# mjmj531/isaacgym

Measured on AMD Instinct MI355X. Metric: env-steps/sec at N_envs=16384 (1/2/4/8 GPUs) + achieved HBM GB/s vs roofline, higher is better.
Workload: dtype f32; 1 GPU; humanoid_pingpong 3-actor tilt (HumanoidPingpongTiltG1), num_envs=16384 per GPU, random U(-1,1) actions, 2 physics substeps per step, fused step kernel; variant=TT, kind=step, num_envs_per_gpu=16384, global_envs=16384, horizon_stats_every=32, prewarm_launches=512, full=False, launch=HIP graph of 32 steps, replayed, parallelism=env-shard x1, no data-path collective

## Files before the change

__graft_entry__.py:

```python
import os
import sys

ROOT = os.path.dirname(os.path.abspath(__file__))
if ROOT not in sys.path:
    sys.path.insert(0, ROOT)


def build():
    from isaacgym_amd import _lib
    _lib.build(force=False)
    from oracle import binding as oracle_binding
    oracle_binding.build()
    sys.path.insert(0, os.path.join(ROOT, "tests"))
    import shim_binding
    shim_binding.lib()
    import dr_shim_binding
    dr_shim_binding.lib()
    import play_shim_binding
    play_shim_binding.lib()
    import ppo_meter_shim_binding
    ppo_meter_shim_binding.lib()
    import urdf_assets
    urdf_assets.build_second_arm_library()
    urdf_assets.build_second_ta_library()
    import isaacgym_amd
    L = _lib.lib()
    from isaacgym_amd import scene
    assert L.ppenv_abi_version() == scene.ABI_VERSION


def smoke():
    import numpy as np
    import torch
    from isaacgym_amd import _lib, scene
    from isaacgym_amd.env import PPEnv
    from oracle import binding as oracle_binding
    sys.path.insert(0, os.path.join(ROOT, "tests"))
    import helpers

    assert torch.cuda.is_available(), "smoke() needs the GPU box"
    _lib.lib()
    n = 256
    cfg = scene.build_config("TT", num_envs=n, seed=1)
    env = PPEnv(scene.build_config("TT", num_envs=n, seed=1), device="cuda:0")
    ora = oracle_binding.OracleEnv(cfg)
    probe = helpers.SensitivityProbe(oracle_binding, cfg)
    oa, ra = helpers.obs_atol(), helpers.reward_atol(cfg)
    rng = np.random.default_rng(0)
    excluded = 0
    for t in range(8):
        a = rng.uniform(-1, 1, (n, 7)).astype(np.float32)
        st = ora.get_state()
        env.set_state(st)
        ora.step(a)
        env.step(torch.from_numpy(a).cuda())
        torch.cuda.synchronize()
        keep = ~probe.sensitive(st, a, ora)
        excluded += int((~keep).sum())
        assert np.array_equal(env.reset_buf.cpu().numpy()[keep], ora.reset_buf[keep])
        helpers.assert_close(env.obs_buf.cpu().numpy()[keep], ora.obs_buf[keep], f"smoke: obs, step {t}", atol=oa)
        helpers.assert_close(env.rew_buf.cpu().numpy()[keep], ora.rew_buf[keep], f"smoke: rew, step {t}", atol=ra)
    assert excluded <= 4, excluded
    assert env.status == 0
    env.close()
    print(f"smoke ok: fused HIP step matches the CPU oracle on {n} envs x 8 steps (rtol 1e-4, the tests' atol; {excluded} env-steps on a switch set aside)")


if __name__ == "__main__":
    build()
    if len(sys.argv) > 1 and sys.argv[1] == "smoke":
        smoke()
```

isaacgym_amd/csrc/ppenv.hip:

```cpp
#include <hip/hip_runtime.h>

#include <algorithm>
#include <cstdio>
#include <cstdlib>
#include <cstring>
#include <new>

using std::min;
using std::max;

#if defined(PP_STAMP)
__device__ unsigned long long pp_stamp_buf[4096 * 32];
#endif
#include "ppenv_device.h"
#include "ppenv_host.h"

using namespace pp;

namespace {

constexpr int kBlock = 64;
constexpr int kObsStride = PPENV_NUM_OBS + 1;
constexpr int kMaxSplitSubsteps = 4;

struct DevBuffers {
    float* obs;
    float* rew;
    long long* reset;
    long long* progress;
    float* dof_pos;
    float* dof_vel;
    float* dof_force;
    float* ball;
    uint32_t* flags;
    uint32_t* episode;
    float* serve;
};

template <class V>
__device__ __forceinline__ void st_state(V* p, V v) { __builtin_nontemporal_store(v, p); }

template <int A>
__device__ __forceinline__ void load_state(const DevBuffers& b, int n, int i, EnvStateT<A>& st) {
#pragma unroll
    for (int d = 0; d < A * ND; d++) {
        st.q[d] = b.dof_pos[(size_t)d * n + i];
        st.qd[d] = b.dof_vel[(size_t)d * n + i];
    }
    float bl[13];
#pragma unroll
    for (int k = 0; k < 13; k++) bl[k] = b.ball[(size_t)k * n + i];
    st.ball.p = mk(bl[0], bl[1], bl[2]);
#pragma unroll
    for (int k = 0; k < 4; k++) st.ball.quat[k] = bl[3 + k];
    st.ball.v = mk(bl[7], bl[8], bl[9]);
    st.ball.w = mk(bl[10], bl[11], bl[12]);
    st.progress = b.progress[(size_t)i * A];
#pragma unroll
    for (int a = 0; a < A; a++) st.flags[a] = b.flags[(size_t)a * n + i];
    st.episode = b.episode[i];
}
__device__ __forceinline__ void store_ball(const DevBuffers& b, int n, int i, const Ball& ball) {
    const float bl[13] = {ball.p.x, ball.p.y, ball.p.z, ball.quat[0], ball.quat[1], ball.quat[2], ball.quat[3],
                          ball.v.x, ball.v.y, ball.v.z, ball.w.x, ball.w.y, ball.w.z};
#pragma unroll
    for (int k = 0; k < 13; k++) st_state(&b.ball[(size_t)k * n + i], bl[k]);
}
template <int A>
__device__ __forceinline__ void store_task(const DevBuffers& b, int n, int i, const EnvStateT<A>& st, const float* rew, long long reset) {
#pragma unroll
    for (int a = 0; a < A; a++) {
        st_state(&b.progress[(size_t)i * A + a], st.progress);
        st_state(&b.flags[(size_t)a * n + i], st.flags[a]);
        st_state(&b.rew[(size_t)i * A + a], rew[a]);
        st_state(&b.reset[(size_t)i * A + a], reset);
    }
    st_state(&b.episode[i], st.episode);
}
template <int A>
__device__ __forceinline__ void store_state(const DevBuffers& b, int n, int i, const EnvStateT<A>& st, const float* rew, long long reset) {
#pragma unroll
    for (int d = 0; d < A * ND; d++) {
        b.dof_pos[(size_t)d * n + i] = st.q[d];
        b.dof_vel[(size_t)d * n + i] = st.qd[d];
        b.dof_force[(size_t)d * n + i] = st.dof_force[d];
    }
    store_ball(b, n, i, st.ball);
    store_task<A>(b, n, i, st, rew, reset);
}

struct LdsRowStore {
    float* row;
    __device__ __forceinline__ void operator()(int k, float v) { row[k] = v; }
};
struct NoisyRowStore {
    float* row;
    float sigma;
    uint64_t seed;
    uint32_t gid, episode, progress;
    uint32_t base = 16u;
    __device__ __forceinline__ void operator()(int k, float v) { row[k] = v + sigma * dr_gauss(seed, gid, episode, progress, base + (uint32_t)k); }
};
struct DRTables {
    const float* kp; const float* kd; const float* ms; const float* es; const float* fs;
    float act_sigma, obs_sigma;
};

__device__ __forceinline__ void flush_obs(const float* s_obs, float* obs, int base, int nvalid, int lane) {
    const int total = nvalid * PPENV_NUM_OBS;
    float4* dst = reinterpret_cast<float4*>(obs + (size_t)base * PPENV_NUM_OBS);
    for (int k = lane * 4; k < total; k += kBlock * 4) {
        int r = k / PPENV_NUM_OBS, c = k - r * PPENV_NUM_OBS;
        const float* src = &s_obs[r * kObsStride + c];
        typedef float f4v __attribute__((ext_vector_type(4)));
        f4v val = {src[0], src[1], src[2], src[3]};
        __builtin_nontemporal_store(val, reinterpret_cast<f4v*>(&dst[k >> 2]));
    }
}

template <class T, bool DR = false>
__global__ __launch_bounds__(kBlock) void step_kernel(const StepConsts K, DevBuffers b, const float* __restrict__ actions, int serve_on, const DRTables drt = DRTables{}) {
    __shared__ float s_obs[kBlock * kObsStride];
    const int lane = threadIdx.x;
    PP_STAMP_AT(0);
    const int n = K.num_envs;
    const int base = blockIdx.x * kBlock;
    const int i = base + lane;
    const int nvalid = min(kBlock, n - base);

    const bool active = i < n;
    EnvState st;
    float rew = 0.f;
    long long reset = 0;
    if (active) {
        float act[ND];
#pragma unroll
        for (int d = 0; d < ND; d++) act[d] = actions[(size_t)i * ND + d];
        load_state<1>(b, n, i, st);
#if defined(PP_STAMP)
        asm volatile("s_waitcnt vmcnt(0) lgkmcnt(0)" ::: "memory");
#endif
        PP_STAMP_AT(1);
        BodyState bodies[NB];
        float pre_vx;
        EnvDR dr;
        const uint32_t gid = (uint32_t)(K.env_id_offset + i), ep0 = st.episode;
        if (DR) {
#pragma unroll
            for (int d = 0; d < ND; d++) {
                dr.kp[d] = drt.kp ? drt.kp[(size_t)d * n + i] : 1.f;
                dr.kd[d] = drt.kd ? drt.kd[(size_t)d * n + i] : 1.f;
                dr.ms[d] = drt.ms ? drt.ms[(size_t)d * n + i] : 1.f;
            }
            dr.es = drt.es ? drt.es[i] : 1.f;
            dr.fs = drt.fs ? drt.fs[i] : 1.f;
            dr.act_sigma = drt.act_sigma; dr.obs_sigma = drt.obs_sigma;
            dr.key_progress = (uint32_t)st.progress;
        }
        simulate_env<T, 1, DR>(K, act, st, bodies, pre_vx, &dr, gid);
        V3 ov = mk(0, 0, 0);
        if (serve_on) ov = mk(b.serve[i], b.serve[(size_t)n + i], b.serve[2 * (size_t)n + i]);
        LdsRowStore store{&s_obs[lane * kObsStride]};
        NoisyRowStore nstore{&s_obs[lane * kObsStride], dr.obs_sigma, K.seed, gid, ep0, dr.key_progress};
        if (DR && drt.obs_sigma > 0.f) post_physics_env<1>(K, gid, st, bodies, pre_vx, serve_on ? &ov : nullptr, &rew, reset, &nstore);
        else post_physics_env<1>(K, gid, st, bodies, pre_vx, serve_on ? &ov : nullptr, &rew, reset, &store);
// ... 855 lines not shown
        hipLaunchKernelGGL((step_kernel_split<ModelG1, 1, 0>), grid, dim3(2 * kBlock), 0, st, e->K, buf, actions_dev, e->serve_on, e->status.dev, e->dbg_drop_handoff);
        break;
    case SCH_FUSED:
        hipLaunchKernelGGL((step_kernel<ModelG1, false>), grid, dim3(kBlock), 0, st, e->K, buf, actions_dev, e->serve_on, DRTables{});
        break;
    }
    PP_HIP(hipGetLastError());
    return PPENV_OK;
}

const char* ppenv_step_kernel_name(ppenv* e) { return e ? kScheduleNames[schedule_of(e)] : ""; }

int ppenv_step(ppenv* e, const float* actions_dev, void* stream) { return launch_step(e, e ? e->buf : DevBuffers{}, actions_dev, stream); }

int ppenv_step_sequence(ppenv* e, const float* const* actions_dev, int32_t count, void* stream) {
    if (!e || !actions_dev || count < 0) { ppenv_set_error("NULL argument or negative count"); return PPENV_EINVAL; }
    for (int32_t i = 0; i < count; i++)
        if (int rc = launch_step(e, e->buf, actions_dev[i], stream)) return rc;
    return PPENV_OK;
}

int ppenv_step_into(ppenv* e, const float* actions_dev, float* obs_dev, float* rew_dev, int64_t* reset_dev, void* stream) {
    if (!e) { ppenv_set_error("NULL argument"); return PPENV_EINVAL; }
    if (obs_dev && (reinterpret_cast<uintptr_t>(obs_dev) & 15)) { ppenv_set_error("ppenv_step_into: obs must be 16-byte aligned"); return PPENV_EINVAL; }
    DevBuffers b = e->buf;
    if (obs_dev) b.obs = obs_dev;
    if (rew_dev) b.rew = rew_dev;
    if (reset_dev) b.reset = reinterpret_cast<long long*>(reset_dev);
    return launch_step(e, b, actions_dev, stream);
}

int ppenv_reset_all(ppenv* e, void* stream) {
    if (!e) { ppenv_set_error("NULL argument"); return PPENV_EINVAL; }
    if (int rc = check_status(e)) return rc;
    if (int rc = pp_use_device(e->cfg.device_id)) return rc;
    launch_init(e, 1, e->serve_on, (hipStream_t)stream);
    PP_HIP(hipGetLastError());
    return PPENV_OK;
}

uint32_t ppenv_status(ppenv* e) { return e ? e->status.read() : 0u; }

int ppenv_set_randomization(ppenv* e, const ppenv_randomization* dr) {
    if (!e) { ppenv_set_error("NULL argument"); return PPENV_EINVAL; }
    if (!dr) { e->dr_on = 0; e->dr = DRTables{}; return PPENV_OK; }
    if (!(dr->action_noise_sigma >= 0.f) || !(dr->observation_noise_sigma >= 0.f)) { ppenv_set_error("noise amplitudes must be >= 0"); return PPENV_EINVAL; }
    e->dr = DRTables{dr->dof_stiffness_scale, dr->dof_damping_scale, dr->link_mass_scale, dr->restitution_scale, dr->friction_scale,
                     dr->action_noise_sigma, dr->observation_noise_sigma};
    e->dr_on = 1;
    return PPENV_OK;
}

int ppenv_set_gravity(ppenv* e, float gravity_z) {
    if (!e) { ppenv_set_error("NULL argument"); return PPENV_EINVAL; }
    if (!(gravity_z <= 0.f)) { ppenv_set_error("gravity_z must be <= 0 (the world's up axis is z)"); return PPENV_EINVAL; }
    e->cfg.gravity_z = gravity_z;
    e->K = make_step_consts(e->cfg);
    return PPENV_OK;
}

int ppenv_reset_idx(ppenv* e, const int64_t* env_ids_dev, int32_t count, int refresh_obs, void* stream) {
    if (!e || (count > 0 && !env_ids_dev) || count < 0) { ppenv_set_error("ppenv_reset_idx: NULL ids or negative count"); return PPENV_EINVAL; }
    if (count == 0) return PPENV_OK;
    if (int rc = check_status(e)) return rc;
    if (int rc = pp_use_device(e->cfg.device_id)) return rc;
    const dim3 grid((count + kBlock - 1) / kBlock), block(kBlock);
    if (e->agents == 2)
        hipLaunchKernelGGL((reset_idx_kernel<ModelG1, 2>), grid, block, 0, (hipStream_t)stream, e->K, e->buf, (const long long*)env_ids_dev, count, refresh_obs, e->serve_on, e->status.dev);
    else
        hipLaunchKernelGGL((reset_idx_kernel<ModelG1, 1>), grid, block, 0, (hipStream_t)stream, e->K, e->buf, (const long long*)env_ids_dev, count, refresh_obs, e->serve_on, e->status.dev);
    PP_HIP(hipGetLastError());
    return PPENV_OK;
}

int ppenv_pd_targets(ppenv* e, const float* actions_dev, float* pd_tar_dev, void* stream) {
    if (!e || !actions_dev || !pd_tar_dev) { ppenv_set_error("NULL argument"); return PPENV_EINVAL; }
    if (int rc = pp_use_device(e->cfg.device_id)) return rc;
    const int rows = e->cfg.num_envs * e->agents;
    hipLaunchKernelGGL(pd_targets_kernel<ModelG1>, dim3((rows * ND + 255) / 256), dim3(256), 0, (hipStream_t)stream, rows, e->K.clip_actions, actions_dev, pd_tar_dev);
    PP_HIP(hipGetLastError());
    return PPENV_OK;
}

int ppenv_serve_from_draws(ppenv* e, const float* draws_dev, int32_t m, float* vel_dev, void* stream) {
    if (!e || !draws_dev || !vel_dev || m <= 0) { ppenv_set_error("NULL argument or m <= 0"); return PPENV_EINVAL; }
    if (int rc = pp_use_device(e->cfg.device_id)) return rc;
    hipLaunchKernelGGL(serve_from_draws_kernel, dim3((m + 255) / 256), dim3(256), 0, (hipStream_t)stream, e->cfg.variant, m, draws_dev, vel_dev);
    PP_HIP(hipGetLastError());
    return PPENV_OK;
}

int ppenv_reduce_stats(ppenv* e, double* out_dev, void* stream) {
    if (!e || !out_dev) { ppenv_set_error("NULL argument"); return PPENV_EINVAL; }
    if (int rc = check_status(e)) return rc;
    if (int rc = pp_use_device(e->cfg.device_id)) return rc;
    const int rows = e->cfg.num_envs * e->agents;
    if (rows <= 32768) {
        hipLaunchKernelGGL(stats_kernel_single, dim3(1), dim3(1024), 0, (hipStream_t)stream, rows, e->agents, e->buf.rew, e->buf.progress,
                           e->buf.episode, out_dev);
    } else {
        PP_HIP(hipMemsetAsync(out_dev, 0, 4 * sizeof(double), (hipStream_t)stream));
        const int blocks = min(256, (rows + 255) / 256);
        hipLaunchKernelGGL(stats_kernel, dim3(blocks), dim3(256), 0, (hipStream_t)stream, rows, e->agents, e->buf.rew, e->buf.progress,
                           e->buf.episode, out_dev);
    }
    PP_HIP(hipGetLastError());
    return PPENV_OK;
}

int ppenv_post_physics_step(ppenv* e, const float* rigid_body_states_dev, float* root_states_dev, float* dof_states_dev,
                            const float* dof_force_dev, const float* pre_ball_vx_dev, void* stream) {
    if (!e || !rigid_body_states_dev || !root_states_dev || !dof_states_dev || !dof_force_dev || !pre_ball_vx_dev) {
        ppenv_set_error("NULL argument");
        return PPENV_EINVAL;
    }
    if (e->agents != 1) { ppenv_set_error("ppenv_post_physics_step serves the 3-actor variants; the 4-actor entry is ppenv_t4_rewards"); return PPENV_EINVAL; }
    if (int rc = check_status(e)) return rc;
    if (int rc = pp_use_device(e->cfg.device_id)) return rc;
    hipLaunchKernelGGL(post_physics_kernel, dim3(grid_for(e->cfg.num_envs)), dim3(kBlock), 0, (hipStream_t)stream, e->K, e->buf,
                       rigid_body_states_dev, root_states_dev, dof_states_dev, dof_force_dev, pre_ball_vx_dev, e->serve_on);
    PP_HIP(hipGetLastError());
    return PPENV_OK;
}

static int refresh(ppenv* e, float* out, void* stream, void (*kernel)(const StepConsts, DevBuffers, float*), int block) {
    if (!e || !out) { ppenv_set_error("NULL argument"); return PPENV_EINVAL; }
    if (int rc = pp_use_device(e->cfg.device_id)) return rc;
    hipLaunchKernelGGL(kernel, dim3((e->cfg.num_envs + block - 1) / block), dim3(block), 0, (hipStream_t)stream, e->K, e->buf, out);
    PP_HIP(hipGetLastError());
    return PPENV_OK;
}
int ppenv_refresh_root_states(ppenv* e, float* out, void* stream) { return refresh(e, out, stream, refresh_root_kernel, 256); }
int ppenv_refresh_dof_states(ppenv* e, float* out, void* stream) { return refresh(e, out, stream, refresh_dof_kernel, 256); }
int ppenv_refresh_dof_force(ppenv* e, float* out, void* stream) { return refresh(e, out, stream, refresh_dof_force_kernel, 256); }
int ppenv_refresh_rigid_body_states(ppenv* e, float* out, void* stream) { return refresh(e, out, stream, refresh_rb_kernel<ModelG1>, kBlock); }

int ppenv_set_serve_override(ppenv* e, const float* serve_dev, int on, void* stream) {
    if (!e) { ppenv_set_error("NULL argument"); return PPENV_EINVAL; }
    if (int rc = pp_use_device(e->cfg.device_id)) return rc;
    if (on && serve_dev) {
        hipLaunchKernelGGL(serve_transpose_kernel, dim3((e->cfg.num_envs + 255) / 256), dim3(256), 0, (hipStream_t)stream, e->cfg.num_envs,
                           serve_dev, e->buf.serve);
        PP_HIP(hipGetLastError());
    }
    e->serve_on = on ? 1 : 0;
    return PPENV_OK;
}

#if defined(PP_STAMP)
int ppenv_debug_read_stamps(unsigned long long* dst, size_t count) {
    if (hipDeviceSynchronize() != hipSuccess) return PPENV_EHIP;
    return hipMemcpyFromSymbol(dst, HIP_SYMBOL(pp_stamp_buf), count * sizeof(unsigned long long)) == hipSuccess ? 0 : PPENV_EHIP;
}
#endif

size_t ppenv_state_bytes(ppenv* e) {
    if (!e) return 0;
    const size_t A = (size_t)e->agents;
    return (size_t)e->cfg.num_envs * ((A * ND * 3 + 13) * 4 + A * 4 + 4 + A * 8 + A * 8);
}

static int state_io(ppenv* e, char* blob, size_t nbytes, bool to_host) {
    if (!e || !blob) { ppenv_set_error("NULL argument"); return PPENV_EINVAL; }
    if (nbytes != ppenv_state_bytes(e)) { ppenv_set_error("state blob size does not match this handle"); return PPENV_ESTATE; }
    if (int rc = pp_use_device(e->cfg.device_id)) return rc;
    PP_HIP(hipDeviceSynchronize());
    if (int rc = check_status(e)) return rc;
    const size_t n = (size_t)e->cfg.num_envs, A = (size_t)e->agents;
    struct Part { void* dev; size_t bytes; };
    const Part parts[] = {{e->buf.dof_pos, n * A * ND * 4}, {e->buf.dof_vel, n * A * ND * 4}, {e->buf.dof_force, n * A * ND * 4}, {e->buf.ball, n * 13 * 4},
                          {e->buf.flags, n * A * 4}, {e->buf.episode, n * 4}, {e->buf.progress, n * A * 8}, {e->buf.reset, n * A * 8}};
    for (const Part& p : parts) {
        if (to_host) PP_HIP(hipMemcpy(blob, p.dev, p.bytes, hipMemcpyDeviceToHost));
        else PP_HIP(hipMemcpy(p.dev, blob, p.bytes, hipMemcpyHostToDevice));
        blob += p.bytes;
    }
    return PPENV_OK;
}
int ppenv_get_state(ppenv* e, void* dst_host, size_t n) { return state_io(e, (char*)dst_host, n, true); }
int ppenv_set_state(ppenv* e, const void* src_host, size_t n) { return state_io(e, (char*)src_host, n, false); }

}
```

isaacgym_amd/csrc/ppenv_device.h:

```cpp
#pragma once

#include <math.h>
#include <stddef.h>
#include <stdint.h>
#include <string.h>

#include "../../include/ppenv.h"

#if defined(__HIPCC__)
#define PP_HD __host__ __device__ __forceinline__
#else
#define PP_HD inline __attribute__((always_inline))
#endif

#if defined(PP_STAMP) && defined(__HIP_DEVICE_COMPILE__)
#define PP_STAMP_AT(k)                                                                      \
    do {                                                                                    \
        __builtin_amdgcn_sched_barrier(0);                                                  \
        unsigned long long t_;                                                              \
        asm volatile("s_memtime %0\n\ts_waitcnt lgkmcnt(0)" : "=s"(t_) : : "memory");      \
        __builtin_amdgcn_sched_barrier(0);                                                  \
        if ((threadIdx.x & 63) == 0) pp_stamp_buf[blockIdx.x * 32 + (k)] = t_;                      \
    } while (0)
extern __device__ unsigned long long pp_stamp_buf[];
// ... 365 lines not shown
                if (FULL) { bodies[j].rot = mul(Rw, ldm(f.origin_rot)); bodies[j].ang = ww; }
            }
        }
    }
};
template <bool FULL>
PP_HD void static_body(const ArmSite& S, BodyState& b) {
    b.pos = ld3(S.root_pos); b.lin = mk(0, 0, 0);
    if (FULL) { b.rot = ldm(S.root_rot); b.ang = mk(0, 0, 0); }
}

template <class T, bool DR = false>
PP_HD void aba_solve(const ArmSite& S, JointSave* js, const float* qd, const float* tau, const float* arm_eff, float* qdd, const EnvDR* dr = nullptr) {
    S3 cA = {0, 0, 0, 0, 0, 0}, cD = {0, 0, 0, 0, 0, 0};
    M3 cB = {{0, 0, 0, 0, 0, 0, 0, 0, 0}};
    V3 cn = mk(0, 0, 0), cf = mk(0, 0, 0);
#pragma unroll
    for (int i = ND - 1; i >= 0; i--) {
        const JointKin JK = T::kin(i);
        const JointInertial J = T::inertial(i);
        const int ax = T::axis(i);
        V3 w = js[i].w, v = js[i].v;
        const float msc = DR ? dr->ms[i] : 1.f;
        float m = DR ? J.mass * msc : J.mass;
        V3 cm = ld3(J.com);
        V3 mc = cm * m;
        float cc = dot(cm, cm);
        float Jin[6];
#pragma unroll
        for (int t = 0; t < 6; t++) Jin[t] = DR ? J.inertia[t] * msc : J.inertia[t];
        S3 A = {Jin[0] + m * (cc - cm.x * cm.x), Jin[1] + m * (cc - cm.y * cm.y), Jin[2] + m * (cc - cm.z * cm.z),
                Jin[3] - m * cm.x * cm.y, Jin[4] - m * cm.x * cm.z, Jin[5] - m * cm.y * cm.z};
        V3 h_ang = mul(A, w) + cross(mc, v);
        V3 h_lin = v * m - cross(mc, w);
        V3 pn = cross(w, h_ang) + cross(v, h_lin) + cn;
        V3 pf = cross(w, h_lin) + cf;
        add_sym(A, cA);
        M3 B = {{cB.m[0], cB.m[1] - mc.z, cB.m[2] + mc.y, cB.m[3] + mc.z, cB.m[4], cB.m[5] - mc.x, cB.m[6] - mc.y, cB.m[7] + mc.x, cB.m[8]}};
        S3 D = {cD.xx + m, cD.yy + m, cD.zz + m, cD.xy, cD.xz, cD.yz};

        V3 ua = symcol(A, ax), ub = row(B, ax);
        float dinv = rcp_fast(symdiag(A, ax) + arm_eff[i]);
        float u = tau[i] - comp(pn, ax);
        js[i].ua = ua; js[i].ub = ub; js[i].dinv = dinv; js[i].u = u;
        if (i > 0) {
            sym_rank1_sub(A, ua, dinv);
            sym_rank1_sub(D, ub, dinv);
            V3 uad = ua * dinv;
#pragma unroll
            for (int r = 0; r < 3; r++) {
                float k = comp(uad, r);
                B.m[3 * r] -= k * ub.x; B.m[3 * r + 1] -= k * ub.y; B.m[3 * r + 2] -= k * ub.z;
            }
            V3 e = unit(ax);
            V3 cw = cross(w, e) * qd[i], cv = cross(v, e) * qd[i];
            float ud = u * dinv;
            V3 pan = pn + mul(A, cw) + mul(B, cv) + ua * ud;
            V3 paf = pf + tmul(B, cw) + mul(D, cv) + ub * ud;
            M3 E = ax == 0 ? joint_rot<0>(JK.origin_rot, js[i].c, js[i].s) : (ax == 1 ? joint_rot<1>(JK.origin_rot, js[i].c, js[i].s) : joint_rot<2>(JK.origin_rot, js[i].c, js[i].s));
            V3 r = ld3(JK.origin_xyz);
            S3 Ar = rot_sym(E, A), Dr = rot_sym(E, D);
            M3 Br = mul_t(mul(E, B), E);
            V3 nr = mul(E, pan), fr = mul(E, paf);
            M3 Dm = from_sym(Dr);
            M3 Bp;
#pragma unroll
            for (int j = 0; j < 3; j++) {
                V3 x = cross(r, col(Dm, j));
                Bp.m[j] = Br.m[j] + x.x; Bp.m[3 + j] = Br.m[3 + j] + x.y; Bp.m[6 + j] = Br.m[6 + j] + x.z;
            }
            V3 wp0 = cross(r, row(Bp, 0)), wp1 = cross(r, row(Bp, 1)), wp2 = cross(r, row(Bp, 2));
            V3 wb0 = cross(r, row(Br, 0)), wb1 = cross(r, row(Br, 1)), wb2 = cross(r, row(Br, 2));
            cA.xx = Ar.xx + wp0.x + wb0.x; cA.yy = Ar.yy + wp1.y + wb1.y; cA.zz = Ar.zz + wp2.z + wb2.z;
            cA.xy = Ar.xy + wp1.x + wb0.y; cA.xz = Ar.xz + wp2.x + wb0.z; cA.yz = Ar.yz + wp2.y + wb1.z;
            cB = Bp; cD = Dr;
            cn = nr + cross(r, fr); cf = fr;
        }
    }
    V3 aw = mk(0, 0, 0);
    V3 av = ld3(S.base_grav);
#pragma unroll
    for (int i = 0; i < ND; i++) {
        const JointKin J = T::kin(i);
        const int ax = T::axis(i);
        M3 E = ax == 0 ? joint_rot<0>(J.origin_rot, js[i].c, js[i].s) : (ax == 1 ? joint_rot<1>(J.origin_rot, js[i].c, js[i].s) : joint_rot<2>(J.origin_rot, js[i].c, js[i].s));
        V3 r = ld3(J.origin_xyz);
        V3 e = unit(ax);
        V3 aw2 = tmul(E, aw) + cross(js[i].w, e) * qd[i];
        V3 av2 = tmul(E, av + cross(aw, r)) + cross(js[i].v, e) * qd[i];
        float a = (js[i].u - dot(js[i].ua, aw2) - dot(js[i].ub, av2)) * js[i].dinv;
        qdd[i] = a;
        if (ax == 0) aw2.x += a; else if (ax == 1) aw2.y += a; else aw2.z += a;
        aw = aw2; av = av2;
    }
}

template <class T, bool DR = false>
PP_HD void arm_substep(const ArmSite& S, JointSave* js, float* q, float* qd, const float* target, float h, float* tau_drive, const EnvDR* dr = nullptr) {
    float tau[ND], arm[ND], qdd[ND];
#pragma unroll
    for (int d = 0; d < ND; d++) {
        const JointDrive J = T::drive(d);
        const float kp = DR ? J.kp * dr->kp[d] : J.kp, kd = DR ? J.kd * dr->kd[d] : J.kd;
        float err = target[d] - q[d];
        tau[d] = fminf(fmaxf(kp * (err - h * qd[d]) - kd * qd[d], -J.effort), J.effort);
        arm[d] = J.armature + h * kd + h * h * kp;
    }
    aba_solve<T, DR>(S, js, qd, tau, arm, qdd, dr);
#pragma unroll
    for (int d = 0; d < ND; d++) {
        const JointDrive J = T::drive(d);
        const float kp = DR ? J.kp * dr->kp[d] : J.kp, kd = DR ? J.kd * dr->kd[d] : J.kd;
        float err = target[d] - q[d];
        float vn = qd[d] + h * qdd[d];
        tau_drive[d] = fminf(fmaxf(kp * (err - h * vn) - kd * vn, -J.effort), J.effort);
        vn = fminf(fmaxf(vn, -J.vel_limit), J.vel_limit);
        float qn = q[d] + h * vn;
        if (qn > J.upper) { qn = J.upper; vn = fminf(vn, 0.f); }
        if (qn < J.lower) { qn = J.lower; vn = fmaxf(vn, 0.f); }
        q[d] = qn; qd[d] = vn;
    }
}

struct Ball { V3 p, v, w; float quat[4]; };

struct BallConsts {
    float contact_offset, bounce_threshold, depen_cap, r;
    float inv_kr;
    float stick_factor;
};

PP_HD void contact_resolve(const BallConsts& k, Ball& b, V3 n, float s, V3 u, float e, float mu) {
    if (!(s < k.contact_offset)) return;
    V3 vrel = b.v + cross(b.w, n * (-k.r)) - u;
    float vn = dot(vrel, n);
    if (vn < 0.f) {
        float e_eff = (-vn > k.bounce_threshold) ? e : 0.f;
        float jn = -(1.f + e_eff) * vn;
        V3 vt = vrel - n * vn;
        float vt2 = dot(vt, vt);
        if (vt2 > 1e-18f) {
            float inv = rsq_fast(vt2);
            V3 dir = vt * inv;
            float jt = fminf(mu * jn, vt2 * inv * k.stick_factor);
            b.v = b.v - dir * jt;
            b.w = b.w + cross(n, dir) * (jt * k.inv_kr);
        }
        b.v = b.v + n * jn;
    }
    if (s < 0.f) b.p = madd(b.p, n, fminf(-s, k.depen_cap));
}
PP_HD float clampf(float x, float lo, float hi) { return fminf(fmaxf(x, lo), hi); }

PP_HD void contact_box(const BallConsts& k, Ball& b, const ppenv_box& box) {
    V3 d = b.p - ld3(box.center);
    V3 h = ld3(box.half);
    float reach = k.r + k.contact_offset;
    if (fabsf(d.x) > h.x + reach || fabsf(d.y) > h.y + reach || fabsf(d.z) > h.z + reach) return;
    V3 q = mk(clampf(d.x, -h.x, h.x), clampf(d.y, -h.y, h.y), clampf(d.z, -h.z, h.z));
    V3 diff = d - q;
    float d2 = dot(diff, diff);
    V3 n;
    float s;
    if (d2 > 1e-24f) { float inv = rsq_fast(d2); n = diff * inv; s = d2 * inv - k.r; }
    else {
        float px = h.x - fabsf(d.x), py = h.y - fabsf(d.y), pz = h.z - fabsf(d.z);
        if (px <= py && px <= pz) { n = mk(d.x >= 0.f ? 1.f : -1.f, 0, 0); s = -px - k.r; }
        else if (py <= pz) { n = mk(0, d.y >= 0.f ? 1.f : -1.f, 0); s = -py - k.r; }
        else { n = mk(0, 0, d.z >= 0.f ? 1.f : -1.f); s = -pz - k.r; }
    }
    contact_resolve(k, b, n, s, mk(0, 0, 0), box.restitution, box.friction);
}
PP_HD void contact_capsule(const BallConsts& k, Ball& b, V3 a, V3 bb, V3 ua, V3 ub, float radius, float e, float mu) {
    V3 ab = bb - a;
    float l2 = dot(ab, ab), t = 0.f;
    if (l2 > 1e-12f) t = clampf(dot(b.p - a, ab) * rcp_fast(l2), 0.f, 1.f);
    V3 cp = madd(a, ab, t);
    V3 diff = b.p - cp;
    float d2 = dot(diff, diff);
    if (d2 > (radius + k.r + k.contact_offset) * (radius + k.r + k.contact_offset)) return;
    float inv = d2 > 1e-24f ? rsq_fast(d2) : 0.f;
    V3 n = d2 > 1e-24f ? diff * inv : mk(0, 0, 1);
    V3 u = madd(ua, ub - ua, t);
    contact_resolve(k, b, n, d2 * inv - radius - k.r, u, e, mu);
}
PP_HD void contact_disc(const BallConsts& k, Ball& b, V3 cc, V3 nn, V3 uc, V3 nd, float R, float tp, float e, float mu) {
    V3 d = b.p - cc;
    float hgt = dot(d, nn);
    V3 radial = d - nn * hgt;
    float rr2 = dot(radial, radial);
    float reach = k.r + k.contact_offset;
    if (fabsf(hgt) > tp + reach || rr2 > (R + reach) * (R + reach)) return;
    float rr = sqrtf(rr2);
    V3 n, closest;
    float s;
    if (fabsf(hgt) < tp && rr < R) {
        float sg = hgt >= 0.f ? 1.f : -1.f;
        n = nn * sg;
        s = -(tp - fabsf(hgt)) - k.r;
        closest = cc + nn * (sg * tp) + radial;
    } else {
        float dh = hgt - clampf(hgt, -tp, tp);
        float er = fmaxf(rr - R, 0.f);
        V3 diff = nn * dh + (er > 0.f ? radial * (er * rcp_fast(rr)) : mk(0, 0, 0));
        closest = b.p - diff;
        float d2 = dh * dh + er * er;
        float inv = d2 > 1e-24f ? rsq_fast(d2) : 0.f;
        n = d2 > 1e-24f ? diff * inv : nn;
        s = d2 * inv - k.r;
    }
    V3 u = uc + cross(cross(nn, nd), closest - cc);
    contact_resolve(k, b, n, s, u, e, mu);
}

PP_HD V3 lerp(V3 a, V3 b, float f) { return madd(a, b - a, f); }

template <class T, int A, bool DR = false>
PP_HD void ball_substep(const StepConsts& K, Ball& b, const ArmGeom<T::kShapes> (&g)[A], const V3 (&bound)[A], const EnvDR* dr = nullptr) {
    const int M = K.ball_substeps;
    const float hb = K.hb, h = K.h;
    BallConsts k;
    k.contact_offset = K.contact_offset;
    k.bounce_threshold = K.bounce_threshold;
    k.depen_cap = K.depen_cap;
    k.r = K.ball_r;
    k.inv_kr = K.inv_kr;
    k.stick_factor = K.stick_factor;
    const float gdv = K.gdv, damp = K.damp;
    const float ground_z = K.ground_z, ground_e = K.ground_e, ground_mu = K.ground_mu;
    const ppenv_box& table = K.table;
    const ppenv_box& net = K.net;
    const ModelPaddle P = T::paddle();
    const float e_cap = K.e_cap;
    const float pad_e = DR ? fminf(K.paddle_e * dr->es, e_cap) : K.paddle_e, pad_mu = DR ? K.paddle_mu * dr->fs : K.paddle_mu;
    const float reach = k.r + k.contact_offset + 1e-4f;
    const float pad_rr = sqrtf(P.radius * P.radius + P.half_thickness * P.half_thickness) + reach;
    const float pad_r2 = pad_rr * pad_rr;
    V3 sc0[A][T::kShapes], svc[A][T::kShapes];
    float sr2[A][T::kShapes];
#pragma unroll
    for (int arm = 0; arm < A; arm++)
#pragma unroll
        for (int s = 0; s < T::kShapes; s++) {
            sc0[arm][s] = (g[arm].a[s] + g[arm].b[s]) * 0.5f;
            svc[arm][s] = (g[arm].va[s] + g[arm].vb[s]) * 0.5f;
            V3 hl = (g[arm].b[s] - g[arm].a[s]) * 0.5f;
            float rr = sqrtf(dot(hl, hl)) + T::shape(s).radius + reach;
            sr2[arm][s] = rr * rr;
        }
    PP_STAMP_AT(26);
    for (int m = 0; m < M; m++) {
        const float t = (float)m * hb;
        PP_STAMP_AT(27 + (m & 3));
        b.v.z += gdv;
        b.w = b.w * damp;
        contact_resolve(k, b, mk(0, 0, 1), b.p.z - ground_z - k.r, mk(0, 0, 0), ground_e, ground_mu);
        contact_box(k, b, table);
        contact_box(k, b, net);
#pragma unroll
        for (int arm = 0; arm < A; arm++) {
            const ArmGeom<T::kShapes>& ga = g[arm];
            V3 db = b.p - bound[arm];
            if (dot(db, db) < K.bound_r2) {
                V3 cc = madd(ga.pc, ga.vpc, t);
                V3 dpc = b.p - cc;
                if (dot(dpc, dpc) < pad_r2) {
                    V3 nn = madd(ga.pn, ga.pnd, t);
                    nn = nn * rsq_fast(dot(nn, nn));
                    contact_disc(k, b, cc, nn, ga.vpc, ga.pnd, P.radius, P.half_thickness, pad_e, pad_mu);
                }
#pragma unroll
                for (int s = 0; s < T::kShapes; s++) {
                    V3 dsc = b.p - madd(sc0[arm][s], svc[arm][s], t);
                    if (dot(dsc, dsc) < sr2[arm][s]) {
                        const float radius = T::shape(s).radius;
                        const float e = DR ? fminf(K.shape_e[s] * dr->es, e_cap) : K.shape_e[s], mu = DR ? K.shape_mu[s] * dr->fs : K.shape_mu[s];
                        if (T::shape_link(s) < 0)
                            contact_capsule(k, b, ga.a[s], ga.b[s], mk(0, 0, 0), mk(0, 0, 0), radius, e, mu);
                        else
                            contact_capsule(k, b, madd(ga.a[s], ga.va[s], t), madd(ga.b[s], ga.vb[s], t), ga.va[s], ga.vb[s], radius, e, mu);
                    }
                }
            }
        }
        b.p = madd(b.p, b.v, hb);
    }
    PP_STAMP_AT(31);
    float wx = b.w.x, wy = b.w.y, wz = b.w.z, x = b.quat[0], y = b.quat[1], z = b.quat[2], w = b.quat[3];
    float kq = 0.5f * h;
    float nx = x + kq * (wx * w + wy * z - wz * y);
    float ny = y + kq * (wy * w + wz * x - wx * z);
    float nz = z + kq * (wz * w + wx * y - wy * x);
    float nw = w + kq * (-wx * x - wy * y - wz * z);
    float inv = rsq_fast(nx * nx + ny * ny + nz * nz + nw * nw);
    b.quat[0] = nx * inv; b.quat[1] = ny * inv; b.quat[2] = nz * inv; b.quat[3] = nw * inv;
}

PP_HD V3 quat_rotate(const float q[4], V3 v) {
    float qw = q[3];
    V3 qv = mk(q[0], q[1], q[2]);
    float s = 2.0f * (qw * qw) - 1.0f;
    V3 cr = cross(qv, v);
    float d = dot(qv, v);
    return mk(v.x * s + cr.x * qw * 2.0f + qv.x * d * 2.0f, v.y * s + cr.y * qw * 2.0f + qv.y * d * 2.0f,
              v.z * s + cr.z * qw * 2.0f + qv.z * d * 2.0f);
}
PP_HD void heading_quat_inv(const float q[4], float out[4]) {
    V3 rd = quat_rotate(q, mk(1, 0, 0));
    float heading = atan2f(rd.y, rd.x);
    float theta = (-heading) / 2.0f;
    float sz = sinf(theta), w = cosf(theta);
    float nrm = fmaxf(sqrtf(sz * sz + w * w), 1e-9f);
    out[0] = 0.f; out[1] = 0.f; out[2] = sz / nrm; out[3] = w / nrm;
}

PP_HD V3 heading_rotate(const float hinv[4], V3 v) {
    float qw = hinv[3], sz = hinv[2];
    float s = 2.0f * (qw * qw) - 1.0f;
    float k = sz * qw * 2.0f;
    return mk(v.x * s - v.y * k, v.y * s + v.x * k, v.z);
}

struct RewardIn {
    float humanoid_x;
    V3 paddle;
    float pre_vx;
    V3 bp;
    float vx;
    float power;
    long long progress;
};

PP_HD float compute_reward(const RewardConsts& c, const RewardIn& in, uint32_t& flags, long long& reset) {
    const float Bx = in.bp.x, By = in.bp.y, Bz = in.bp.z, vx = in.vx, pre_vx = in.pre_vx;
    const float alpha = c.alpha, penalty = c.penalty, threshold = 0.1f;
    const float power_reward = -c.power_coefficient * in.power;
    const int variant = c.variant;
    uint32_t f = flags;
    float reward;
    long long die = 0;
    if (variant == PPENV_VARIANT_T3) {
        V3 dp = in.paddle - in.bp;
        float dist = sqrtf(dp.x * dp.x + dp.y * dp.y + dp.z * dp.z);
        float pos_reward = 1.0f / (1.0f + 1.5f * dist * dist);
        float vel_reward = (pre_vx < 0.f && vx > 0.f) ? alpha * fabsf(vx) : 0.f;
        reward = pos_reward + power_reward + vel_reward;
        bool missed = Bx < in.paddle.x - 1e-3f;
        if (missed) { reward = reward + penalty; die = 1; }
        if (Bz < threshold) die = 1;
    } else if (variant == PPENV_VARIANT_TT || variant == PPENV_VARIANT_T4) {
        V3 dp = in.paddle - in.bp;
        float dist = sqrtf(dp.x * dp.x + dp.y * dp.y + dp.z * dp.z);
        float pos_reward = 1.0f / (1.0f + 1.5f * dist * dist);
        bool cond = pre_vx < 0.f && vx > 0.f;
        float vel_reward = (cond && !(f & PPENV_FLAG_COND_CALC)) ? alpha * fabsf(vx) : 0.f;
        if (cond) f |= PPENV_FLAG_COND_CALC;
        bool missed = Bx < in.humanoid_x - 0.05f;
        reward = missed ? 0.f + penalty : 0.f;
        bool bounce = Bz < 0.83f && vx > 0.f && By < 0.6f && By > -0.6f;
        float hit = 0.f;
        bool early = Bx < 2.44f && bounce;
        if (early && !(f & PPENV_FLAG_REWARD_CALC)) hit = c.not_hit_table_penalty;
        if (early) { f |= PPENV_FLAG_REWARD_CALC; f &= ~PPENV_FLAG_NO_BOUNCE; }
        bool inx = Bx > 2.44f && Bx < 3.1f;
        bool good = inx && bounce && (f & PPENV_FLAG_NO_BOUNCE);
        if (good && !(f & PPENV_FLAG_REWARD_CALC)) hit = c.hit_table_reward;
        if (good) f |= PPENV_FLAG_REWARD_CALC;
        if (Bx >= 3.1f && vx > 0.f && !(f & PPENV_FLAG_REWARD_CALC)) hit = c.not_hit_table_penalty;
        if (Bx >= 3.1f) f |= PPENV_FLAG_REWARD_CALC;
        float net = (Bx > 1.7f && Bx < 1.8f && vx > 0.f && By < 0.4f && By > -0.4f && Bz > 0.98f && Bz < 1.14f) ? 400.f : 0.f;
        reward += (((pos_reward + power_reward) + vel_reward) + hit) + net;
        if (Bz < threshold) die = 1;
    } else {
        bool hit_paddle = pre_vx < 0.f && vx > 1.0f;
        bool missed = (Bx < in.humanoid_x - 0.05f) || (Bx < in.paddle.x - 0.1f);
        reward = (!(f & PPENV_FLAG_MISSED_CALC) && missed) ? 0.f + penalty : 0.f;
        if (missed) f |= PPENV_FLAG_MISSED_CALC;
        float dy = in.paddle.y - By, dz = in.paddle.z - Bz;
        float dist = sqrtf(dy * dy + dz * dz);
        float pos_reward = 0.f;
        if (!(f & PPENV_FLAG_COND_CALC) || (Bx < in.humanoid_x - 0.05f)) pos_reward = 1.0f * expf(-20.0f * dist * dist);
        float vel_reward = (hit_paddle && !(f & PPENV_FLAG_COND_CALC)) ? alpha * fabsf(vx) : 0.f;
        if (hit_paddle) f |= PPENV_FLAG_COND_CALC;
        reward += (pos_reward + power_reward) + vel_reward;
        if (Bz < threshold) reward = -800.f + reward;
    }
    flags = f;
    reset = (in.progress >= (long long)c.max_episode_length - 1) ? 1 : die;
    return reward;
}

PP_HD float compute_reward_side2(const RewardConsts& c, const RewardIn& in, uint32_t& flags, long long& reset) {
    const float Bx = in.bp.x, By = in.bp.y, Bz = in.bp.z, vx = in.vx, pre_vx = in.pre_vx;
    uint32_t f = flags;
    V3 dp = in.paddle - in.bp;
    float dist = sqrtf(dp.x * dp.x + dp.y * dp.y + dp.z * dp.z);
    float pos_reward = 1.0f / (1.0f + 1.5f * dist * dist);
    bool cond = pre_vx > 0.f && vx < 0.f;
    float vel_reward = (cond && !(f & PPENV_FLAG_COND_CALC)) ? c.alpha * fabsf(vx) : 0.f;
    if (cond) f |= PPENV_FLAG_COND_CALC;
    bool missed = Bx > in.humanoid_x + 0.05f;
    float reward = missed ? 0.f + c.penalty : 0.f;
    bool bounce = Bz < 0.83f && vx < 0.f && By < 0.6f && By > -0.6f;
    float hit = 0.f;
    bool early = Bx > 1.06f && bounce;
    if (early && !(f & PPENV_FLAG_REWARD_CALC)) hit = c.not_hit_table_penalty;
    if (early) { f |= PPENV_FLAG_REWARD_CALC; f &= ~PPENV_FLAG_NO_BOUNCE; }
    bool inx = Bx < 1.06f && Bx > 0.4f;
    bool good = inx && bounce && (f & PPENV_FLAG_NO_BOUNCE);
    if (good && !(f & PPENV_FLAG_REWARD_CALC)) hit = c.hit_table_reward;
    if (good) f |= PPENV_FLAG_REWARD_CALC;
    if (Bx <= 0.4f && vx < 0.f && !(f & PPENV_FLAG_REWARD_CALC)) hit = c.not_hit_table_penalty;
    if (Bx <= 0.4f) f |= PPENV_FLAG_REWARD_CALC;
    float net = (Bx > 1.7f && Bx < 1.8f && vx < 0.f && By < 0.4f && By > -0.4f && Bz > 0.98f && Bz < 1.14f) ? 400.f : 0.f;
    float power_reward = -c.power_coefficient * in.power;
    reward += (((pos_reward + power_reward) + vel_reward) + hit) + net;
    flags = f;
    reset = (in.progress >= (long long)c.max_episode_length - 1) ? 1 : (Bz < 0.1f ? 1 : 0);
    return reward;
}

template <int A>
struct EnvStateT {
    float q[A * ND], qd[A * ND], dof_force[A * ND];
    Ball ball;
    long long progress;
    uint32_t flags[A], episode;
};
using EnvState = EnvStateT<1>;

template <class T, int A, bool DR = false>
PP_HD void simulate_env(const StepConsts& K, const float* actions, EnvStateT<A>& st, BodyState* bodies, float& pre_vx, const EnvDR* dr = nullptr, uint32_t gid = 0) {
    float target[A * ND];
#pragma unroll
    for (int d = 0; d < A * ND; d++) {
        float act = actions[d];
        if (DR) { if (dr->act_sigma > 0.f) act += dr->act_sigma * dr_gauss(K.seed, gid, st.episode, dr->key_progress, (uint32_t)d); }
// ... 251 lines not shown
```

Before: 1.393 billion env-steps/s.

## Split ball contact pass into detect-then-resolve with sequential fallback

Ball contact handling in each substep now runs as a detection pass. The pass records the first contact and flags whether a second contact or a nearby shape (within the depenetration growth margin) could be affected. Only lanes flagged this way rerun the original sequential resolve from the next shape index, and the rerun is skipped when no lane in the wavefront needs it. The goal is to stop calling contact_resolve inline for every shape and to shorten the divergent per-shape work, at the cost of extra conservative 'near' distance checks and a possible second pass when a wavefront has multi-contact lanes. A compile-time switch keeps the old sequential path, and debug path counters are added under PP_STAMP.

```diff
diff --git a/__graft_entry__.py b/__graft_entry__.py
--- a/__graft_entry__.py
+++ b/__graft_entry__.py
@@ -23,6 +23,8 @@
     import urdf_assets
     urdf_assets.build_second_arm_library()
     urdf_assets.build_second_ta_library()
+    import ball_variant
+    ball_variant.build_ball_sequential_library()
     import isaacgym_amd
     L = _lib.lib()
     from isaacgym_amd import scene
diff --git a/isaacgym_amd/csrc/ppenv.hip b/isaacgym_amd/csrc/ppenv.hip
--- a/isaacgym_amd/csrc/ppenv.hip
+++ b/isaacgym_amd/csrc/ppenv.hip
@@ -11,6 +11,7 @@
 
 #if defined(PP_STAMP)
 __device__ unsigned long long pp_stamp_buf[4096 * 32];
+__device__ unsigned int pp_ball_paths[8];
 #endif
 #include "ppenv_device.h"
 #include "ppenv_host.h"
@@ -1172,6 +1173,12 @@
     if (hipDeviceSynchronize() != hipSuccess) return PPENV_EHIP;
     return hipMemcpyFromSymbol(dst, HIP_SYMBOL(pp_stamp_buf), count * sizeof(unsigned long long)) == hipSuccess ? 0 : PPENV_EHIP;
 }
+int ppenv_debug_read_ball_paths(unsigned int* dst ) {
+    static const unsigned int zero[8] = {0};
+    if (hipDeviceSynchronize() != hipSuccess) return PPENV_EHIP;
+    if (hipMemcpyFromSymbol(dst, HIP_SYMBOL(pp_ball_paths), sizeof zero) != hipSuccess) return PPENV_EHIP;
+    return hipMemcpyToSymbol(HIP_SYMBOL(pp_ball_paths), zero, sizeof zero) == hipSuccess ? 0 : PPENV_EHIP;
+}
 #endif
 
 size_t ppenv_state_bytes(ppenv* e) {
diff --git a/isaacgym_amd/csrc/ppenv_device.h b/isaacgym_amd/csrc/ppenv_device.h
--- a/isaacgym_amd/csrc/ppenv_device.h
+++ b/isaacgym_amd/csrc/ppenv_device.h
@@ -541,11 +541,18 @@
 }
 PP_HD float clampf(float x, float lo, float hi) { return fminf(fmaxf(x, lo), hi); }
 
-PP_HD void contact_box(const BallConsts& k, Ball& b, const ppenv_box& box) {
-    V3 d = b.p - ld3(box.center);
+struct Contact { V3 n; float s; V3 u; float e, mu; };
+PP_HD void contact_resolve(const BallConsts& k, Ball& b, const Contact& c) { contact_resolve(k, b, c.n, c.s, c.u, c.e, c.mu); }
+
+PP_HD bool contact_ground(const BallConsts& k, V3 p, float ground_z, float e, float mu, Contact& c) {
+    c.n = mk(0, 0, 1); c.s = p.z - ground_z - k.r; c.u = mk(0, 0, 0); c.e = e; c.mu = mu;
+    return c.s < k.contact_offset;
+}
+PP_HD bool contact_box(const BallConsts& k, V3 p, const ppenv_box& box, Contact& c) {
+    V3 d = p - ld3(box.center);
     V3 h = ld3(box.half);
     float reach = k.r + k.contact_offset;
-    if (fabsf(d.x) > h.x + reach || fabsf(d.y) > h.y + reach || fabsf(d.z) > h.z + reach) return;
+    if (fabsf(d.x) > h.x + reach || fabsf(d.y) > h.y + reach || fabsf(d.z) > h.z + reach) return false;
     V3 q = mk(clampf(d.x, -h.x, h.x), clampf(d.y, -h.y, h.y), clampf(d.z, -h.z, h.z));
     V3 diff = d - q;
     float d2 = dot(diff, diff);
@@ -558,28 +565,30 @@
         else if (py <= pz) { n = mk(0, d.y >= 0.f ? 1.f : -1.f, 0); s = -py - k.r; }
         else { n = mk(0, 0, d.z >= 0.f ? 1.f : -1.f); s = -pz - k.r; }
     }
-    contact_resolve(k, b, n, s, mk(0, 0, 0), box.restitution, box.friction);
-}
-PP_HD void contact_capsule(const BallConsts& k, Ball& b, V3 a, V3 bb, V3 ua, V3 ub, float radius, float e, float mu) {
+    c.n = n; c.s = s; c.u = mk(0, 0, 0); c.e = box.restitution; c.mu = box.friction;
+    return s < k.contact_offset;
+}
+PP_HD bool contact_capsule(const BallConsts& k, V3 p, V3 a, V3 bb, V3 ua, V3 ub, float radius, float e, float mu, Contact& c) {
     V3 ab = bb - a;
     float l2 = dot(ab, ab), t = 0.f;
-    if (l2 > 1e-12f) t = clampf(dot(b.p - a, ab) * rcp_fast(l2), 0.f, 1.f);
+    if (l2 > 1e-12f) t = clampf(dot(p - a, ab) * rcp_fast(l2), 0.f, 1.f);
     V3 cp = madd(a, ab, t);
-    V3 diff = b.p - cp;
+    V3 diff = p - cp;
     float d2 = dot(diff, diff);
-    if (d2 > (radius + k.r + k.contact_offset) * (radius + k.r + k.contact_offset)) return;
+    if (d2 > (radius + k.r + k.contact_offset) * (radius + k.r + k.contact_offset)) return false;
     float inv = d2 > 1e-24f ? rsq_fast(d2) : 0.f;
-    V3 n = d2 > 1e-24f ? diff * inv : mk(0, 0, 1);
-    V3 u = madd(ua, ub - ua, t);
-    contact_resolve(k, b, n, d2 * inv - radius - k.r, u, e, mu);
-}
-PP_HD void contact_disc(const BallConsts& k, Ball& b, V3 cc, V3 nn, V3 uc, V3 nd, float R, float tp, float e, float mu) {
-    V3 d = b.p - cc;
+    c.n = d2 > 1e-24f ? diff * inv : mk(0, 0, 1);
+    c.u = madd(ua, ub - ua, t);
+    c.s = d2 * inv - radius - k.r; c.e = e; c.mu = mu;
+    return c.s < k.contact_offset;
+}
+PP_HD bool contact_disc(const BallConsts& k, V3 p, V3 cc, V3 nn, V3 uc, V3 nd, float R, float tp, float e, float mu, Contact& c) {
+    V3 d = p - cc;
     float hgt = dot(d, nn);
     V3 radial = d - nn * hgt;
     float rr2 = dot(radial, radial);
     float reach = k.r + k.contact_offset;
-    if (fabsf(hgt) > tp + reach || rr2 > (R + reach) * (R + reach)) return;
+    if (fabsf(hgt) > tp + reach || rr2 > (R + reach) * (R + reach)) return false;
     float rr = sqrtf(rr2);
     V3 n, closest;
     float s;
@@ -592,17 +601,119 @@
         float dh = hgt - clampf(hgt, -tp, tp);
         float er = fmaxf(rr - R, 0.f);
         V3 diff = nn * dh + (er > 0.f ? radial * (er * rcp_fast(rr)) : mk(0, 0, 0));
-        closest = b.p - diff;
+        closest = p - diff;
         float d2 = dh * dh + er * er;
         float inv = d2 > 1e-24f ? rsq_fast(d2) : 0.f;
         n = d2 > 1e-24f ? diff * inv : nn;
         s = d2 * inv - k.r;
     }
-    V3 u = uc + cross(cross(nn, nd), closest - cc);
-    contact_resolve(k, b, n, s, u, e, mu);
+    c.n = n; c.s = s; c.u = uc + cross(cross(nn, nd), closest - cc); c.e = e; c.mu = mu;
+    return s < k.contact_offset;
 }
 
 PP_HD V3 lerp(V3 a, V3 b, float f) { return madd(a, b - a, f); }
+
+#ifndef PP_BALL_SEQUENTIAL
+#define PP_BALL_SEQUENTIAL 0
+#endif
+#if defined(__HIP_DEVICE_COMPILE__)
+#define PP_WAVE_ANY(x) (__builtin_amdgcn_ballot_w64(x) != 0ull)
+#else
+#define PP_WAVE_ANY(x) (x)
+#endif
+#if !defined(PP_BALL_PATH)
+#if defined(PP_STAMP) && defined(__HIP_DEVICE_COMPILE__)
+extern __device__ unsigned int pp_ball_paths[8];
+#define PP_BALL_PATH(hit, again)                                                                                   \
+    do {                                                                                                           \
+        const unsigned long long mh_ = __builtin_amdgcn_ballot_w64(hit), ma_ = __builtin_amdgcn_ballot_w64(again);  \
+        if ((threadIdx.x & 63) == 0) {                                                                             \
+            atomicAdd(&pp_ball_paths[0], 1u);                                                                      \
+            atomicAdd(&pp_ball_paths[1], mh_ != 0ull ? 1u : 0u);                                                   \
+            atomicAdd(&pp_ball_paths[2], ma_ != 0ull ? 1u : 0u);                                                   \
+            atomicAdd(&pp_ball_paths[3], (unsigned int)__builtin_popcountll(mh_));                                 \
+            atomicAdd(&pp_ball_paths[4], (unsigned int)__builtin_popcountll(ma_));                                 \
+        }                                                                                                          \
+    } while (0)
+#else
+#define PP_BALL_PATH(hit, again) do { } while (0)
+#endif
+#endif
+
+template <class T, int A>
+struct BallShapes {
+    V3 sc0[A][T::kShapes], svc[A][T::kShapes];
+    float sr2[A][T::kShapes];
+    float sr2_far[A][T::kShapes];
+    float pad_e, pad_mu, pad_r2, pad_r2_far, bound_r2_far;
+    float grow;
+};
+PP_HD bool box_within(V3 p, const ppenv_box& box, float reach) {
+    V3 d = p - ld3(box.center);
+    V3 h = ld3(box.half);
+    return !(fabsf(d.x) > h.x + reach || fabsf(d.y) > h.y + reach || fabsf(d.z) > h.z + reach);
+}
+
+struct Paths { int first; bool second, near; };
+template <bool SEQ>
+PP_HD void contact_take(const BallConsts& k, Ball& b, const Contact& c, int idx, Paths& w, Contact& hit) {
+    if (SEQ) contact_resolve(k, b, c);
+    else if (w.first < 0) { hit = c; w.first = idx; }
+    else w.second = true;
+}
+
+template <class T, int A, bool DR, bool SEQ>
+PP_HD void ball_contacts(const StepConsts& K, const BallConsts& k, const BallShapes<T, A>& S, const ArmGeom<T::kShapes> (&g)[A], const V3 (&bound)[A],
+                         const EnvDR* dr, float t, Ball& b, Paths& w, Contact& hit) {
+    const ModelPaddle P = T::paddle();
+    const int from = w.first;
+    const float box_far = k.r + k.contact_offset + S.grow;
+    Contact c;
+    if (!SEQ || from < 0) { if (contact_ground(k, b.p, K.ground_z, K.ground_e, K.ground_mu, c)) contact_take<SEQ>(k, b, c, 0, w, hit); }
+    if (!SEQ && w.first >= 0) w.near = w.near || box_within(b.p, K.table, box_far);
+    if (!SEQ || from < 1) { if (contact_box(k, b.p, K.table, c)) contact_take<SEQ>(k, b, c, 1, w, hit); }
+    if (!SEQ && w.first >= 0) w.near = w.near || box_within(b.p, K.net, box_far);
+    if (!SEQ || from < 2) { if (contact_box(k, b.p, K.net, c)) contact_take<SEQ>(k, b, c, 2, w, hit); }
+#pragma unroll
+    for (int arm = 0; arm < A; arm++) {
+        const ArmGeom<T::kShapes>& ga = g[arm];
+        const int i0 = 3 + arm * (1 + T::kShapes);
+        if (SEQ && from >= i0 + T::kShapes) continue;
+        const bool inside = SEQ && from >= i0;
+        V3 db = b.p - bound[arm];
+        const float db2 = dot(db, db);
+        if (!SEQ && w.first >= 0 && !(db2 < K.bound_r2) && db2 < S.bound_r2_far) w.near = true;
+        if (inside || db2 < K.bound_r2) {
+            if (!SEQ || from < i0) {
+                V3 cc = madd(ga.pc, ga.vpc, t);
+                V3 dpc = b.p - cc;
+                const float dpc2 = dot(dpc, dpc);
+                if (!SEQ && w.first >= 0 && dpc2 < S.pad_r2_far) w.near = true;
+                if (dpc2 < S.pad_r2) {
+                    V3 nn = madd(ga.pn, ga.pnd, t);
+                    nn = nn * rsq_fast(dot(nn, nn));
+                    if (contact_disc(k, b.p, cc, nn, ga.vpc, ga.pnd, P.radius, P.half_thickness, S.pad_e, S.pad_mu, c))
+                        contact_take<SEQ>(k, b, c, i0, w, hit);
+                }
+            }
+#pragma unroll
+            for (int s = 0; s < T::kShapes; s++) {
+                if (SEQ && from >= i0 + 1 + s) continue;
+                V3 dsc = b.p - madd(S.sc0[arm][s], S.svc[arm][s], t);
+                const float dsc2 = dot(dsc, dsc);
+                if (!SEQ && w.first >= 0 && dsc2 < S.sr2_far[arm][s]) w.near = true;
+                if (dsc2 < S.sr2[arm][s]) {
+                    const float radius = T::shape(s).radius;
+                    const float e = DR ? fminf(K.shape_e[s] * dr->es, K.e_cap) : K.shape_e[s], mu = DR ? K.shape_mu[s] * dr->fs : K.shape_mu[s];
+                    const bool touch = T::shape_link(s) < 0
+                        ? contact_capsule(k, b.p, ga.a[s], ga.b[s], mk(0, 0, 0), mk(0, 0, 0), radius, e, mu, c)
+                        : contact_capsule(k, b.p, madd(ga.a[s], ga.va[s], t), madd(ga.b[s], ga.vb[s], t), ga.va[s], ga.vb[s], radius, e, mu, c);
+                    if (touch) contact_take<SEQ>(k, b, c, i0 + 1 + s, w, hit);
+                }
+            }
+        }
+    }
+}
 
 template <class T, int A, bool DR = false>
 PP_HD void ball_substep(const StepConsts& K, Ball& b, const ArmGeom<T::kShapes> (&g)[A], const V3 (&bound)[A], const EnvDR* dr = nullptr) {
@@ -616,26 +727,28 @@
     k.inv_kr = K.inv_kr;
     k.stick_factor = K.stick_factor;
     const float gdv = K.gdv, damp = K.damp;
-    const float ground_z = K.ground_z, ground_e = K.ground_e, ground_mu = K.ground_mu;
-    const ppenv_box& table = K.table;
-    const ppenv_box& net = K.net;
     const ModelPaddle P = T::paddle();
     const float e_cap = K.e_cap;
-    const float pad_e = DR ? fminf(K.paddle_e * dr->es, e_cap) : K.paddle_e, pad_mu = DR ? K.paddle_mu * dr->fs : K.paddle_mu;
+    BallShapes<T, A> S;
+    S.pad_e = DR ? fminf(K.paddle_e * dr->es, e_cap) : K.paddle_e;
+    S.pad_mu = DR ? K.paddle_mu * dr->fs : K.paddle_mu;
     const float reach = k.r + k.contact_offset + 1e-4f;
     const float pad_rr = sqrtf(P.radius * P.radius + P.half_thickness * P.half_thickness) + reach;
-    const float pad_r2 = pad_rr * pad_rr;
-    V3 sc0[A][T::kShapes], svc[A][T::kShapes];
-    float sr2[A][T::kShapes];
+    S.pad_r2 = pad_rr * pad_rr;
+    S.grow = k.depen_cap + 1e-4f;
+    S.pad_r2_far = (pad_rr + S.grow) * (pad_rr + S.grow);
+    const float bound_far = sqrtf(K.bound_r2) + S.grow;
+    S.bound_r2_far = bound_far * bound_far;
 #pragma unroll
     for (int arm = 0; arm < A; arm++)
 #pragma unroll
         for (int s = 0; s < T::kShapes; s++) {
-            sc0[arm][s] = (g[arm].a[s] + g[arm].b[s]) * 0.5f;
-            svc[arm][s] = (g[arm].va[s] + g[arm].vb[s]) * 0.5f;
+            S.sc0[arm][s] = (g[arm].a[s] + g[arm].b[s]) * 0.5f;
+            S.svc[arm][s] = (g[arm].va[s] + g[arm].vb[s]) * 0.5f;
             V3 hl = (g[arm].b[s] - g[arm].a[s]) * 0.5f;
             float rr = sqrtf(dot(hl, hl)) + T::shape(s).radius + reach;
-            sr2[arm][s] = rr * rr;
+            S.sr2[arm][s] = rr * rr;
+            S.sr2_far[arm][s] = (rr + S.grow) * (rr + S.grow);
         }
     PP_STAMP_AT(26);
     for (int m = 0; m < M; m++) {
@@ -643,35 +756,19 @@
         PP_STAMP_AT(27 + (m & 3));
         b.v.z += gdv;
         b.w = b.w * damp;
-        contact_resolve(k, b, mk(0, 0, 1), b.p.z - ground_z - k.r, mk(0, 0, 0), ground_e, ground_mu);
-        contact_box(k, b, table);
-        contact_box(k, b, net);
-#pragma unroll
-        for (int arm = 0; arm < A; arm++) {
-            const ArmGeom<T::kShapes>& ga = g[arm];
-            V3 db = b.p - bound[arm];
-            if (dot(db, db) < K.bound_r2) {
-                V3 cc = madd(ga.pc, ga.vpc, t);
-                V3 dpc = b.p - cc;
-                if (dot(dpc, dpc) < pad_r2) {
-                    V3 nn = madd(ga.pn, ga.pnd, t);
-                    nn = nn * rsq_fast(dot(nn, nn));
-                    contact_disc(k, b, cc, nn, ga.vpc, ga.pnd, P.radius, P.half_thickness, pad_e, pad_mu);
-                }
-#pragma unroll
-                for (int s = 0; s < T::kShapes; s++) {
-                    V3 dsc = b.p - madd(sc0[arm][s], svc[arm][s], t);
-                    if (dot(dsc, dsc) < sr2[arm][s]) {
-                        const float radius = T::shape(s).radius;
-                        const float e = DR ? fminf(K.shape_e[s] * dr->es, e_cap) : K.shape_e[s], mu = DR ? K.shape_mu[s] * dr->fs : K.shape_mu[s];
-                        if (T::shape_link(s) < 0)
-                            contact_capsule(k, b, ga.a[s], ga.b[s], mk(0, 0, 0), mk(0, 0, 0), radius, e, mu);
-                        else
-                            contact_capsule(k, b, madd(ga.a[s], ga.va[s], t), madd(ga.b[s], ga.vb[s], t), ga.va[s], ga.vb[s], radius, e, mu);
-                    }
-                }
-            }
+        Paths w = {-1, false, false};
+        Contact hit;
+#if PP_BALL_SEQUENTIAL
+        ball_contacts<T, A, DR, true>(K, k, S, g, bound, dr, t, b, w, hit);
+#else
+        ball_contacts<T, A, DR, false>(K, k, S, g, bound, dr, t, b, w, hit);
+        if (w.first >= 0) contact_resolve(k, b, hit);
+        const bool again = w.first >= 0 && (w.second || (w.near && hit.s < 0.f));
+        PP_BALL_PATH(w.first >= 0, again);
+        if (PP_WAVE_ANY(again)) {
+            if (again) ball_contacts<T, A, DR, true>(K, k, S, g, bound, dr, t, b, w, hit);
         }
+#endif
         b.p = madd(b.p, b.v, hb);
     }
     PP_STAMP_AT(31);
```

After: 1.110 billion env-steps/s. -20.3%, worse.
